# yxgeee/OpenIBL

Measured on NVIDIA H100. Metric: images_per_sec_extraction, higher is better.
Workload: dtype f32 (bf16x3 split on wgmma, fp32 accumulate)

## Files before the change

### openibl_b200/csrc/tc_conv.cu

```cuda
#include "common.cuh"
#include "tc_common.cuh"

namespace ibl {

using namespace tc;

namespace tc {
EncodeTiledFn get_encode_tiled() {
  static const EncodeTiledFn fn = []() -> EncodeTiledFn {
    void* p = nullptr;
    cudaDriverEntryPointQueryResult qres;
    if (cudaGetDriverEntryPoint("cuTensorMapEncodeTiled", &p, cudaEnableDefault, &qres) ==
            cudaSuccess &&
        qres == cudaDriverEntryPointSuccess)
      return reinterpret_cast<EncodeTiledFn>(p);
    return nullptr;
  }();
  return fn;
}

int make_tmap(CUtensorMap* out, CUtensorMapDataType dt, int rank, const void* base,
              const uint64_t* dims, const uint64_t* strides_bytes, const uint32_t* box, int swizzle_bytes) {
  EncodeTiledFn enc = get_encode_tiled();
  if (!enc) {
// ... 13 lines not shown
                   CU_TENSOR_MAP_INTERLEAVE_NONE,
                   swizzle_bytes == 64 ? CU_TENSOR_MAP_SWIZZLE_64B : CU_TENSOR_MAP_SWIZZLE_128B,
                   CU_TENSOR_MAP_L2_PROMOTION_L2_256B, CU_TENSOR_MAP_FLOAT_OOB_FILL_NONE);
  if (r != CUDA_SUCCESS) {
    set_last_error("cuTensorMapEncodeTiled failed with CUresult " + std::to_string((int)r));
    return IBL_ERR_CUDA;
  }
  return IBL_OK;
}
}

int tc_driver_init() { return get_encode_tiled() ? IBL_OK : IBL_ERR_NO_DEVICE; }

struct ConvTcArgs {
  int N, H, W, cin, cout;
  int tw_log2;
  int tiles_w, tiles_h;
  int n_tiles;
  int total_tiles;
  int relu, pool;
  const float* bias;
  __nv_bfloat16* y_hi;
  __nv_bfloat16* y_lo;
  float* y_f32;
  float* ssq;
  long long ssq_stride;
};

__device__ __forceinline__ uint32_t pack_bf16x2(float a, float b) {
  __nv_bfloat162 t = __floats2bfloat162_rn(a, b);
  return *reinterpret_cast<uint32_t*>(&t);
}

template <int BN>
__device__ __forceinline__ void conv_epilogue_tile(const ConvTcArgs& a, const Acc128<BN>& acc, float* stg, int img, int h0,
                                                   int w0, int n0, int nt, int r, int c, int dr_lanes, int bar = 1) {
  const int h = h0 + r, w = w0 + c;
  bool valid;
  long long pix;
  if (a.pool) {
    const int OH = a.H >> 1, OW = a.W >> 1;
    const int oh = h >> 1, ow = w >> 1;
    valid = oh < OH && ow < OW && img < a.N;
    pix = ((long long)img * OH + oh) * OW + ow;
  } else {
    valid = h < a.H && w < a.W && img < a.N;
    pix = ((long long)img * a.H + h) * a.W + w;
  }
  float ssq_acc = 0.f;
#pragma unroll
  for (int ch = 0; ch < BN / 32; ++ch) {
    uint32_t raw[32];
    acc.rows32(ch, stg, raw, bar);
    if (a.pool) {
      const bool s1 = (c & 1) != 0, s2 = (r & 1) != 0;
      float u[16];
#pragma unroll
      for (int j = 0; j < 16; ++j) {
        const float lo_h = __uint_as_float(raw[j]), hi_h = __uint_as_float(raw[j + 16]);
        const float got = __shfl_xor_sync(0xffffffffu, s1 ? lo_h : hi_h, 1);
        u[j] = fmaxf(s1 ? hi_h : lo_h, got);
      }
      float w8[8];
#pragma unroll
      for (int j = 0; j < 8; ++j) {
        const float got = __shfl_xor_sync(0xffffffffu, s2 ? u[j] : u[j + 8], dr_lanes);
        w8[j] = fmaxf(s2 ? u[j + 8] : u[j], got);
      }
      if (valid) {
        const int cbase = n0 + ch * 32 + (s1 ? 16 : 0) + (s2 ? 8 : 0);
        const float4 b0 = __ldg(reinterpret_cast<const float4*>(a.bias + cbase));
        const float4 b1 = __ldg(reinterpret_cast<const float4*>(a.bias + cbase) + 1);
        const float bb[8] = {b0.x, b0.y, b0.z, b0.w, b1.x, b1.y, b1.z, b1.w};
#pragma unroll
        for (int j = 0; j < 8; ++j) {
          w8[j] = w8[j] + bb[j];
          if (a.relu) w8[j] = fmaxf(w8[j], 0.f);
        }
        const long long off = pix * a.cout + cbase;
        if (a.y_f32) {
          float4* o = reinterpret_cast<float4*>(a.y_f32 + off);
          o[0] = make_float4(w8[0], w8[1], w8[2], w8[3]);
          o[1] = make_float4(w8[4], w8[5], w8[6], w8[7]);
        } else {
          uint32_t hi[4], lo[4];
#pragma unroll
          for (int j = 0; j < 4; ++j) {
            const float x0 = w8[2 * j], x1 = w8[2 * j + 1];
            const __nv_bfloat16 h0b = __float2bfloat16_rn(x0), h1b = __float2bfloat16_rn(x1);
            __nv_bfloat162 hh(h0b, h1b);
            hi[j] = *reinterpret_cast<uint32_t*>(&hh);
            lo[j] = pack_bf16x2(x0 - __bfloat162float(h0b), x1 - __bfloat162float(h1b));
          }
          *reinterpret_cast<uint4*>(a.y_hi + off) = make_uint4(hi[0], hi[1], hi[2], hi[3]);
          *reinterpret_cast<uint4*>(a.y_lo + off) = make_uint4(lo[0], lo[1], lo[2], lo[3]);
        }
      }
      continue;
    }
    float v[32];
    const float4* bp = reinterpret_cast<const float4*>(a.bias + n0 + ch * 32);
#pragma unroll
    for (int j = 0; j < 8; ++j) {
      const float4 b = __ldg(bp + j);
      v[4 * j + 0] = __uint_as_float(raw[4 * j + 0]) + b.x;
      v[4 * j + 1] = __uint_as_float(raw[4 * j + 1]) + b.y;
      v[4 * j + 2] = __uint_as_float(raw[4 * j + 2]) + b.z;
      v[4 * j + 3] = __uint_as_float(raw[4 * j + 3]) + b.w;
    }
    if (a.relu) {
#pragma unroll
      for (int j = 0; j < 32; ++j) v[j] = fmaxf(v[j], 0.f);
    }
    if (a.ssq) {
#pragma unroll
      for (int j = 0; j < 32; ++j) ssq_acc = fmaf(v[j], v[j], ssq_acc);
    }
    if (valid) {
      const long long off = pix * a.cout + n0 + ch * 32;
      if (a.y_f32) {
        float4* o = reinterpret_cast<float4*>(a.y_f32 + off);
#pragma unroll
        for (int j = 0; j < 8; ++j) o[j] = make_float4(v[4 * j], v[4 * j + 1], v[4 * j + 2], v[4 * j + 3]);
      } else {
        uint32_t hi[16], lo[16];
#pragma unroll
        for (int j = 0; j < 16; ++j) {
          const float x0 = v[2 * j], x1 = v[2 * j + 1];
          const __nv_bfloat16 h0b = __float2bfloat16_rn(x0), h1b = __float2bfloat16_rn(x1);
          __nv_bfloat162 hh(h0b, h1b);
          hi[j] = *reinterpret_cast<uint32_t*>(&hh);
          lo[j] = pack_bf16x2(x0 - __bfloat162float(h0b), x1 - __bfloat162float(h1b));
        }
        uint4* oh4 = reinterpret_cast<uint4*>(a.y_hi + off);
        uint4* ol4 = reinterpret_cast<uint4*>(a.y_lo + off);
#pragma unroll
        for (int j = 0; j < 4; ++j) {
          oh4[j] = make_uint4(hi[4 * j], hi[4 * j + 1], hi[4 * j + 2], hi[4 * j + 3]);
          ol4[j] = make_uint4(lo[4 * j], lo[4 * j + 1], lo[4 * j + 2], lo[4 * j + 3]);
        }
      }
    }
  }
  if (a.ssq && valid && !a.pool) a.ssq[(long long)nt * a.ssq_stride + pix] = ssq_acc;
}

constexpr int TC_BM = 128;
constexpr int TC_BK = 64;
constexpr int TC_A_BYTES = TC_BM * TC_BK * 2;

constexpr int TC_HALO_W = 10, TC_HALO_H = 18;
constexpr int TC_HALO_ROWS = TC_HALO_W * TC_HALO_H;
constexpr int TC_HALO_PLANE = 23 * 1024;
constexpr int TC_HALO_STAGE = 2 * TC_HALO_PLANE;

constexpr int TC_WIDE_PX = 256;
constexpr int TC_WIDE_HALO_PLANE = 41 * 1024;

template <int BN, int STAGES, bool HALO = false, int NA = 0, int WTW = 0>
struct ConvTcSmem {
  static constexpr int THREADS = HALO ? 384 : 160;
  static constexpr int CONSUMERS = HALO ? 2 : 1;
  static constexpr int B_BYTES = BN * TC_BK * 2;
  static constexpr int STAGE_BYTES = HALO ? 2 * B_BYTES : 2 * TC_A_BYTES + 2 * B_BYTES;
  static constexpr int HALO_PLANE = WTW ? TC_WIDE_HALO_PLANE : TC_HALO_PLANE;
  static constexpr int A_RING = HALO ? NA * 2 * HALO_PLANE : 0;
  static constexpr int STG = WTW ? 0 : CONSUMERS * ACC_STG_BYTES;
  static constexpr int BYTES = A_RING + STAGES * STAGE_BYTES + STG + 1024  + 256 ;
};

struct AccWide {
  float d[2][64];
};

__device__ __forceinline__ float wide_pick(bool swap, float a, float b) { return swap ? b : a; }

__device__ __forceinline__ void wide_transpose4(uint32_t (&x)[4][2], int j) {
#pragma unroll
  for (int bit = 0; bit < 2; ++bit) {
    const bool mine = ((j >> bit) & 1) != 0;
#pragma unroll
    for (int p0 = 0; p0 < 4; ++p0) {
      if (p0 & (1 << bit)) continue;
      const int p1 = p0 | (1 << bit);
#pragma unroll
      for (int h = 0; h < 2; ++h) {
        const uint32_t got = __shfl_xor_sync(0xffffffffu, mine ? x[p0][h] : x[p1][h], 4 << bit);
        if (mine) x[p0][h] = got; else x[p1][h] = got;
      }
    }
  }
}

__device__ __forceinline__ void conv_wide_epilogue(const ConvTcArgs& a, const AccWide& acc, int img, int h0, int w0,
                                                   int nt) {
  constexpr int NV = 2, TH = 16;
  const int t = threadIdx.x & 127, w = t >> 5, lane = t & 31, g = lane >> 2, q = lane & 3, j = g & 3;
  const bool sw = (g >> 2) != 0;
  const int c = nt * 64 + 16 * w + 2 * g;
  const int cst = nt * 64 + 16 * w + 8 * (g >> 2);
  const float b0 = __ldg(a.bias + c), b1 = __ldg(a.bias + c + 1);
  auto activate = [&](float& v0, float& v1) {
    v0 += b0; v1 += b1;
    if (a.relu) { v0 = fmaxf(v0, 0.f); v1 = fmaxf(v1, 0.f); }
  };
  auto pack = [&](float v0, float v1, uint32_t (&x)[2]) {
    if (a.y_f32) {
      x[0] = __float_as_uint(v0); x[1] = __float_as_uint(v1);
    } else {
      const __nv_bfloat16 h0b = __float2bfloat16_rn(v0), h1b = __float2bfloat16_rn(v1);
      __nv_bfloat162 hh(h0b, h1b);
      x[0] = *reinterpret_cast<uint32_t*>(&hh);
      x[1] = pack_bf16x2(v0 - __bfloat162float(h0b), v1 - __bfloat162float(h1b));
    }
  };
  auto store = [&](const uint32_t (&x)[4][2], bool valid, long long pix) {
    if (!valid) return;
    const long long off = pix * a.cout + cst;
    if (a.y_f32) {
      float4* o = reinterpret_cast<float4*>(a.y_f32 + off);
      o[0] = make_float4(__uint_as_float(x[0][0]), __uint_as_float(x[0][1]), __uint_as_float(x[1][0]), __uint_as_float(x[1][1]));
      o[1] = make_float4(__uint_as_float(x[2][0]), __uint_as_float(x[2][1]), __uint_as_float(x[3][0]), __uint_as_float(x[3][1]));
    } else {
      *reinterpret_cast<uint4*>(a.y_hi + off) = make_uint4(x[0][0], x[1][0], x[2][0], x[3][0]);
      *reinterpret_cast<uint4*>(a.y_lo + off) = make_uint4(x[0][1], x[1][1], x[2][1], x[3][1]);
    }
  };
  if (a.pool) {
    const int OH = a.H >> 1, OW = a.W >> 1;
    const int ow = (w0 >> 1) + q;
#pragma unroll
    for (int v = 0; v < NV; ++v)
#pragma unroll
      for (int m = 0; m < TH / 8; ++m) {
        uint32_t x[4][2];
#pragma unroll
        for (int p = 0; p < 4; ++p) {
          const float* r0 = &acc.d[v][4 * (2 * (4 * m + p))];
          const float* r1 = r0 + 4;
          const float e0 = fmaxf(fmaxf(r0[0], r0[1]), fmaxf(r1[0], r1[1]));
          const float e1 = fmaxf(fmaxf(r0[2], r0[3]), fmaxf(r1[2], r1[3]));
          float v0 = wide_pick(sw, e0, e1), v1 = wide_pick(sw, e1, e0);
          activate(v0, v1);
          pack(v0, v1, x[p]);
        }
        wide_transpose4(x, j);
        const int oh = (h0 >> 1) + 4 * m + j, owv = ow + 4 * v;
        store(x, oh < OH && owv < OW && img < a.N, ((long long)img * OH + oh) * OW + owv);
      }
    return;
  }
#pragma unroll
  for (int v = 0; v < NV; ++v)
#pragma unroll
    for (int b = 0; b < TH / 2; ++b) {
      uint32_t x[4][2];
      float sq[4];
#pragma unroll
      for (int p = 0; p < 4; ++p) {
        const float* r = &acc.d[v][4 * (2 * b + (p >> 1)) + (p & 1)];
        const float e0 = r[0], e1 = r[2];
        float v0 = wide_pick(sw, e0, e1), v1 = wide_pick(sw, e1, e0);
        activate(v0, v1);
        sq[p] = fmaf(v1, v1, v0 * v0);
        pack(v0, v1, x[p]);
      }
      wide_transpose4(x, j);
      const int h = h0 + 2 * b + (j >> 1), wc = w0 + 8 * v + 2 * q + (j & 1);
      const bool valid = h < a.H && wc < a.W && img < a.N;
      const long long pix = ((long long)img * a.H + h) * a.W + wc;
      store(x, valid, pix);
      if (a.ssq) {
        float mine = 0.f;
#pragma unroll
        for (int p = 0; p < 4; ++p) {
          float s2 = sq[p];
          s2 += __shfl_xor_sync(0xffffffffu, s2, 4);
          s2 += __shfl_xor_sync(0xffffffffu, s2, 8);
          s2 += __shfl_xor_sync(0xffffffffu, s2, 16);
          if (p == j) mine = s2;
        }
        if (valid && g < 4) a.ssq[(long long)(nt * 4 + w) * a.ssq_stride + pix] = mine;
      }
    }
}

template <int BN, int STAGES, bool HALO, int NA, int WTW = 0>
__global__ void __launch_bounds__(ConvTcSmem<BN, STAGES, HALO, NA, WTW>::THREADS, 1)
conv3x3_tc_kernel(const __grid_constant__ CUtensorMap tm_xhi, const __grid_constant__ CUtensorMap tm_xlo,
                  const __grid_constant__ CUtensorMap tm_whi, const __grid_constant__ CUtensorMap tm_wlo,
                  const ConvTcArgs a) {
  extern __shared__ __align__(1024) uint8_t smem_raw[];
  uint8_t* smem = reinterpret_cast<uint8_t*>((reinterpret_cast<uintptr_t>(smem_raw) + 1023) & ~uintptr_t(1023));
  using L = ConvTcSmem<BN, STAGES, HALO, NA, WTW>;
  constexpr int HALO_PLANE = L::HALO_PLANE;
  constexpr int HALO_STAGE = 2 * HALO_PLANE;
  constexpr int PX = WTW ? TC_WIDE_PX : TC_BM;
  constexpr int B_BYTES = L::B_BYTES;
  constexpr int STAGE_BYTES = L::STAGE_BYTES;
  constexpr int A_RING = L::A_RING;
  uint8_t* ring = smem + A_RING;
  float* stg = reinterpret_cast<float*>(ring + STAGES * STAGE_BYTES);
  uint64_t* bars = reinterpret_cast<uint64_t*>(ring + STAGES * STAGE_BYTES + L::STG);
  uint64_t* full_bar = bars;
  uint64_t* empty_bar = bars + STAGES;
  uint64_t* afull_bar = bars + 2 * STAGES;
  uint64_t* aempty_bar = afull_bar + NA;
// ... 245 lines not shown
#pragma unroll
          for (int k = 0; k < TC_BK / 16; ++k) {
            const uint64_t ko = (uint64_t)(k * 2);
            acc.mma(a_lo + ko, a_lo + a_half + ko, b_hi + ko, (kc > 0 || tap > 0 || k > 0) ? 1u : 0u);
            acc.mma(a_hi + ko, a_hi + a_half + ko, b_lo + ko, 1u);
            acc.mma(a_hi + ko, a_hi + a_half + ko, b_hi + ko, 1u);
          }
          wgmma_commit();
          if (kc == kchunks - 1 && tap == 8 && lane == 0) mbar_arrive(&order_bar[cw ^ 1]);
          wgmma_wait<1>();
          if (prev >= 0) release_w(prev);
          if (prev_a >= 0) {
            if (lane == 0) mbar_arrive(&aempty_bar[prev_a]);
            prev_a = -1;
          }
          prev = stage;
          if (++stage == STAGES) { stage = 0; phase ^= 1; }
        }
        prev_a = astage;
        if (++astage == NA) { astage = 0; aphase ^= 1; }
      }
      wgmma_wait<0>();
      acc.fence_operands();
      release_w(prev);
      if (lane == 0) mbar_arrive(&aempty_bar[prev_a]);
      conv_epilogue_tile<BN>(a, acc, my_stg, img, h0, w0, nt * BN, nt, r, c, 8, bar);
    }
    } else {
    const int m = threadIdx.x;
    const int r = m >> a.tw_log2, c = m & (TW - 1);
    int stage = 0;
    uint32_t phase = 0;
    for (int tile = worker; tile < a.total_tiles; tile += n_workers) {
      int img, h0, w0, nt;
      coords(tile, img, h0, w0, nt);
      Acc128<BN> acc;
      int prev = -1;
      for (int kit = 0; kit < kiters; ++kit) {
        mbar_wait(&full_bar[stage], phase);
        const uint32_t sa = ring_a + stage * STAGE_BYTES;
        const uint64_t a_hi = gmma_desc_kmajor_sw128(sa), a_lo = gmma_desc_kmajor_sw128(sa + TC_A_BYTES);
        const uint64_t b_hi = gmma_desc_kmajor_sw128(sa + 2 * TC_A_BYTES);
        const uint64_t b_lo = gmma_desc_kmajor_sw128(sa + 2 * TC_A_BYTES + B_BYTES);
        constexpr uint64_t kHalf = (TC_BM / 2) * 128 / 16;
        wgmma_fence();
#pragma unroll
        for (int k = 0; k < TC_BK / 16; ++k) {
          const uint64_t ko = (uint64_t)(k * 2);
          acc.mma(a_lo + ko, a_lo + kHalf + ko, b_hi + ko, (kit > 0 || k > 0) ? 1u : 0u);
          acc.mma(a_hi + ko, a_hi + kHalf + ko, b_lo + ko, 1u);
          acc.mma(a_hi + ko, a_hi + kHalf + ko, b_hi + ko, 1u);
        }
        wgmma_commit();
        wgmma_wait<1>();
        if (prev >= 0) release_w(prev);
        prev = stage;
        if (++stage == STAGES) { stage = 0; phase ^= 1; }
      }
      wgmma_wait<0>();
      acc.fence_operands();
      if (prev >= 0) release_w(prev);
      conv_epilogue_tile<BN>(a, acc, stg, img, h0, w0, nt * BN, nt, r, c, TW);
    }
    }
  }
  __syncthreads();
}

template <int BN, int STAGES, bool HALO = false, int NA = 0, int WTW = 0>
static int launch_tc_variant(const CUtensorMap& xhi, const CUtensorMap& xlo, const CUtensorMap& whi,
                             const CUtensorMap& wlo, const ConvTcArgs& a, cudaStream_t s) {
  constexpr int smem = ConvTcSmem<BN, STAGES, HALO, NA, WTW>::BYTES;
  static_assert(smem <= 232448, "shared-memory budget");
  static DeviceOnce attr_done;
  if (!attr_done.done()) {
    IBL_CUDA_OK(cudaFuncSetAttribute(conv3x3_tc_kernel<BN, STAGES, HALO, NA, WTW>,
                                     cudaFuncAttributeMaxDynamicSharedMemorySize, smem));
    attr_done.mark();
  }
  const int sms = device_sm_count();
  const int grid = a.total_tiles < sms ? a.total_tiles : sms;
  conv3x3_tc_kernel<BN, STAGES, HALO, NA, WTW>
      <<<grid, ConvTcSmem<BN, STAGES, HALO, NA, WTW>::THREADS, smem, s>>>(xhi, xlo, whi, wlo, a);
  IBL_CUDA_OK(cudaGetLastError());
  return IBL_OK;
}

static int g_tc_bn_override = 0;
void tc_set_bn_override(int bn) { g_tc_bn_override = bn; }
static int g_tc_variant_override = 0;
void tc_set_variant_override(int v) { g_tc_variant_override = v; }

int launch_conv3x3_tc(const __nv_bfloat16* x_hi, const __nv_bfloat16* x_lo, const ConvParams& p,
                      int N, int H, int W, int cin, int cout, bool relu, bool pool,
                      __nv_bfloat16* y_hi, __nv_bfloat16* y_lo, float* y_f32, cudaStream_t s, float* ssq,
                      int* ssq_parts) {
  IBL_REQUIRE(cin % 64 == 0 && cout % 64 == 0, "tensor-core conv needs Cin%64==0 and Cout%64==0");
  IBL_REQUIRE(p.w_hi && p.w_lo, "tensor-core conv: weights were not re-laid-out");
  IBL_REQUIRE(H >= 1 && W >= 1 && N >= 1, "empty conv input");
  ConvTcArgs a{};
  a.N = N; a.H = H; a.W = W; a.cin = cin; a.cout = cout;
  auto waste = [&](int tw, int px) {
    int th = px / tw;
    return (long long)cdiv(W, tw) * tw * cdiv(H, th) * th;
  };
  const int tw128 = (waste(16, 128) <= waste(8, 128)) ? 16 : 8;
  constexpr int tw256 = 16;
  bool wide = waste(tw256, 256) <= waste(tw128, 128);
  if (g_tc_bn_override) wide = false;
  if (g_tc_variant_override) wide = g_tc_variant_override == 2;
  const int TW = wide ? tw256 : tw128, TH = (wide ? TC_WIDE_PX : TC_BM) / TW;
  a.tw_log2 = TW == 16 ? 4 : 3;
  a.tiles_w = cdiv(W, TW);
  a.tiles_h = cdiv(H, TH);
  int bn = wide ? 64 : cout % 128 == 0 ? 128 : 64;
  if (!wide && g_tc_bn_override && cout % g_tc_bn_override == 0 && (g_tc_bn_override == 64 || g_tc_bn_override == 128))
    bn = g_tc_bn_override;
  const bool halo = wide || bn == 128;
  a.n_tiles = cout / bn;
  a.total_tiles = (int)((long long)N * a.tiles_h * a.tiles_w * a.n_tiles);
  a.relu = relu; a.pool = pool;
  a.bias = p.bias; a.y_hi = y_hi; a.y_lo = y_lo; a.y_f32 = y_f32;
  a.ssq = pool ? nullptr : ssq;
  a.ssq_stride = (long long)N * H * W;
  if (ssq_parts) *ssq_parts = wide ? cout / 16 : a.n_tiles;

  CUtensorMap m_xhi, m_xlo, m_whi, m_wlo;
  {
    uint64_t dims[4] = {(uint64_t)cin, (uint64_t)W, (uint64_t)H, (uint64_t)N};
    uint64_t str[3] = {(uint64_t)cin * 2, (uint64_t)W * cin * 2, (uint64_t)H * W * cin * 2};
    uint32_t box[4] = {64, (uint32_t)(halo ? TW + 2 : TW), (uint32_t)(halo ? TH + 2 : TH), 1};
    IBL_RET(make_tmap(&m_xhi, CU_TENSOR_MAP_DATA_TYPE_BFLOAT16, 4, x_hi, dims, str, box));
    IBL_RET(make_tmap(&m_xlo, CU_TENSOR_MAP_DATA_TYPE_BFLOAT16, 4, x_lo, dims, str, box));
  }
  {
    uint64_t dims[3] = {(uint64_t)cin, (uint64_t)cout, 9};
    uint64_t str[2] = {(uint64_t)cin * 2, (uint64_t)cout * cin * 2};
    uint32_t box[3] = {64, (uint32_t)bn, 1};
    IBL_RET(make_tmap(&m_whi, CU_TENSOR_MAP_DATA_TYPE_BFLOAT16, 3, p.w_hi, dims, str, box));
    IBL_RET(make_tmap(&m_wlo, CU_TENSOR_MAP_DATA_TYPE_BFLOAT16, 3, p.w_lo, dims, str, box));
  }
  if (wide) return launch_tc_variant<64, 3, true, 2, 16>(m_xhi, m_xlo, m_whi, m_wlo, a, s);
  if (halo) return launch_tc_variant<128, 3, true, 2>(m_xhi, m_xlo, m_whi, m_wlo, a, s);
  return launch_tc_variant<64, 4>(m_xhi, m_xlo, m_whi, m_wlo, a, s);
}

struct Conv1FusedArgs {
  const float* x;
  const float* w1;
  const float* bias1;
  ConvTcArgs c2;
};

constexpr int F1_A1_ROWS = 192;
constexpr int F1_A1_PLANE = F1_A1_ROWS * 64;
constexpr int F1_W1_PLANE = 64 * 64;
constexpr int F1_W2_STAGE = 2 * 64 * TC_BK * 2;
constexpr int F1_W2_STAGES = 4;
constexpr int F1_OFF_W1 = 2 * TC_HALO_STAGE;
constexpr int F1_OFF_W2 = F1_OFF_W1 + 2 * F1_W1_PLANE;
constexpr int F1_OFF_STG = F1_OFF_W2 + F1_W2_STAGES * F1_W2_STAGE;
constexpr int F1_OFF_BAR = F1_OFF_STG + 2 * ACC_STG_BYTES;
constexpr int F1_SMEM = F1_OFF_BAR + 512 + 1024;
static_assert(2 * F1_A1_PLANE <= TC_HALO_STAGE, "A1 (hi | lo) is built inside the consumer's halo buffer");
static_assert(TC_HALO_STAGE % 1024 == 0 && F1_OFF_W1 % 512 == 0 && F1_OFF_W2 % 1024 == 0, "swizzle atom alignment");
static_assert(F1_SMEM <= 232448, "shared-memory budget of the fused conv1 kernel");

__device__ __forceinline__ void wgmma_n64_into_n128(float (&d)[64], uint64_t a, uint64_t b) {
  asm volatile(
      "{\n\t.reg .pred p;\n\tsetp.ne.b32 p, 1, 0;\n\t"
      "wgmma.mma_async.sync.aligned.m64n64k16.f32.bf16.bf16 {%0, %1, %2, %3, %4, %5, %6, %7, %8, %9, %10, %11, %12, %13, %14, %15, %16, %17, %18, %19, %20, %21, %22, %23, %24, %25, %26, %27, %28, %29, %30, %31}, %32, %33, p, 1, 1, 0, 0;\n\t}"
      : "+f"(d[0]), "+f"(d[1]), "+f"(d[2]), "+f"(d[3]), "+f"(d[4]), "+f"(d[5]), "+f"(d[6]), "+f"(d[7]), "+f"(d[8]), "+f"(d[9]), "+f"(d[10]), "+f"(d[11]), "+f"(d[12]), "+f"(d[13]), "+f"(d[14]), "+f"(d[15]), "+f"(d[16]), "+f"(d[17]), "+f"(d[18]), "+f"(d[19]), "+f"(d[20]), "+f"(d[21]), "+f"(d[22]), "+f"(d[23]), "+f"(d[24]), "+f"(d[25]), "+f"(d[26]), "+f"(d[27]), "+f"(d[28]), "+f"(d[29]), "+f"(d[30]), "+f"(d[31])
      : "l"(a), "l"(b));
}

__global__ void __launch_bounds__(384, 1)
conv1_fused_tc_kernel(const __grid_constant__ CUtensorMap tm_whi, const __grid_constant__ CUtensorMap tm_wlo,
                      const Conv1FusedArgs fa) {
  extern __shared__ __align__(1024) uint8_t smem_raw[];
  uint8_t* smem = reinterpret_cast<uint8_t*>((reinterpret_cast<uintptr_t>(smem_raw) + 1023) & ~uintptr_t(1023));
  const ConvTcArgs& a = fa.c2;
  uint8_t* w1 = smem + F1_OFF_W1;
  uint8_t* w2 = smem + F1_OFF_W2;
  float* stg = reinterpret_cast<float*>(smem + F1_OFF_STG);
  uint64_t* bars = reinterpret_cast<uint64_t*>(smem + F1_OFF_BAR);
  uint64_t* w_full = bars;
  uint64_t* w_empty = bars + F1_W2_STAGES;
  uint64_t* order_bar = bars + 2 * F1_W2_STAGES;
  float* bias1_s = reinterpret_cast<float*>(bars + 16);

  const int warp = threadIdx.x >> 5, lane = threadIdx.x & 31;
  for (int i = threadIdx.x; i < 64 * 4; i += blockDim.x) {
    const int n = i >> 2, j = i & 3;
    uint32_t hi[4], lo[4];
#pragma unroll
    for (int e = 0; e < 4; ++e) {
      float v[2];
#pragma unroll
      for (int u = 0; u < 2; ++u) {
        const int k = j * 8 + e * 2 + u;
        v[u] = 0.f;
        if (k < 27) v[u] = fa.w1[(n * 3 + (k % 3)) * 9 + (k / 3)];
      }
      const __nv_bfloat16 h0 = __float2bfloat16_rn(v[0]), h1 = __float2bfloat16_rn(v[1]);
      __nv_bfloat162 hh(h0, h1);
      hi[e] = *reinterpret_cast<uint32_t*>(&hh);
      lo[e] = pack_bf16x2(v[0] - __bfloat162float(h0), v[1] - __bfloat162float(h1));
    }
    const int pos = n * 64 + ((j ^ ((n >> 1) & 3)) * 16);
    *reinterpret_cast<uint4*>(w1 + pos) = make_uint4(hi[0], hi[1], hi[2], hi[3]);
    *reinterpret_cast<uint4*>(w1 + F1_W1_PLANE + pos) = make_uint4(lo[0], lo[1], lo[2], lo[3]);
  }
  if (threadIdx.x < 64) bias1_s[threadIdx.x] = fa.bias1[threadIdx.x];
  if (threadIdx.x == 0) {
    tma_prefetch_desc(&tm_whi);
    tma_prefetch_desc(&tm_wlo);
    for (int i = 0; i < F1_W2_STAGES; ++i) { mbar_init(&w_full[i], 1); mbar_init(&w_empty[i], 4); }
    mbar_init(&order_bar[0], 4);
    mbar_init(&order_bar[1], 4);
    fence_barrier_init();
  }
  fence_proxy_async();
  __syncthreads();
  const int tiles_per_img = a.tiles_h * a.tiles_w;
  auto coords = [&](int tile, int& img, int& h0, int& w0) {
    img = tile / tiles_per_img;
    const int rem = tile - img * tiles_per_img;
    h0 = (rem / a.tiles_w) * 16;
    w0 = (rem % a.tiles_w) * 8;
  };

  if (warp < 4) setmaxnreg_dec<40>();
  if (warp == 0) {
    int stage = 0; uint32_t phase = 0;
    for (int tile = blockIdx.x; tile < a.total_tiles; tile += gridDim.x) {
      for (int tap = 0; tap < 9; ++tap) {
        mbar_wait_warp(&w_empty[stage], phase ^ 1);
        uint8_t* st = w2 + stage * F1_W2_STAGE;
        if (elect_one()) {
          mbar_arrive_expect_tx(&w_full[stage], F1_W2_STAGE);
          tma_load_3d(st, &tm_whi, &w_full[stage], 0, 0, tap);
          tma_load_3d(st + F1_W2_STAGE / 2, &tm_wlo, &w_full[stage], 0, 0, tap);
        }
        __syncwarp();
        if (++stage == F1_W2_STAGES) { stage = 0; phase ^= 1; }
      }
    }
  } else if (warp >= 4) {
    setmaxnreg_inc<232>();
    const int cw = warp / 4 - 1;
    const int bar = 1 + cw;
    float* my_stg = stg + cw * (ACC_STG_BYTES / 4);
    uint8_t* halo = smem + cw * TC_HALO_STAGE;
    const int t = threadIdx.x & 127;
    const int r = t >> 3, c = t & 7;
    const uint32_t ha = smem_u32(halo);
    const uint64_t b1h = gmma_desc_kmajor_sw64(smem_u32(w1)), b1l = gmma_desc_kmajor_sw64(smem_u32(w1) + F1_W1_PLANE);
    const uint64_t a1h = gmma_desc_kmajor_sw64(ha), a1l = gmma_desc_kmajor_sw64(ha + F1_A1_PLANE);
    constexpr uint64_t kA1Tile = 64 * 64 / 16;
    constexpr uint64_t kHaloDesc = ((uint64_t)1 << 16) | ((uint64_t)((TC_HALO_W * 128) >> 4) << 32) | ((uint64_t)1 << 62);
    constexpr uint64_t kHaloHalf = 8 * TC_HALO_W * 128 / 16;
    const long long HW = (long long)a.H * a.W;
    for (int i = cw; blockIdx.x + i * gridDim.x < a.total_tiles; i += 2) {
      int img, h0, w0;
      coords(blockIdx.x + i * gridDim.x, img, h0, w0);
      int tl = t;
      asm volatile("" : "+r"(tl));
#pragma unroll
      for (int q = 0; q < 2; ++q) {
        const int p = q * 128 + tl;
        if (p < F1_A1_ROWS) {
          float v[32];
#pragma unroll
          for (int k = 0; k < 32; ++k) v[k] = 0.f;
          const int hl = p / TC_HALO_W, wl = p - hl * TC_HALO_W;
          const int ph = h0 - 1 + hl, pw = w0 - 1 + wl;
          if (p < TC_HALO_ROWS && ph >= 0 && ph < a.H && pw >= 0 && pw < a.W && img < a.N) {
            const float* xb = fa.x + (long long)img * 3 * HW;
#pragma unroll
            for (int tap = 0; tap < 9; ++tap) {
              const int ih = ph + tap / 3 - 1, iw = pw + tap % 3 - 1;
              if (ih >= 0 && ih < a.H && iw >= 0 && iw < a.W) {
                const long long o = (long long)ih * a.W + iw;
#pragma unroll
                for (int ci = 0; ci < 3; ++ci) v[tap * 3 + ci] = __ldg(xb + ci * HW + o);
              }
            }
          }
          uint8_t* rh = halo + p * 64;
#pragma unroll
          for (int j = 0; j < 4; ++j) {
            uint32_t hi[4], lo[4];
#pragma unroll
            for (int e = 0; e < 4; ++e) {
              const float x0 = v[8 * j + 2 * e], x1 = v[8 * j + 2 * e + 1];
              const __nv_bfloat16 h0b = __float2bfloat16_rn(x0), h1b = __float2bfloat16_rn(x1);
              __nv_bfloat162 hv(h0b, h1b);
              hi[e] = *reinterpret_cast<uint32_t*>(&hv);
              lo[e] = pack_bf16x2(x0 - __bfloat162float(h0b), x1 - __bfloat162float(h1b));
            }
            const int pos = (j ^ ((p >> 1) & 3)) * 16;
            *reinterpret_cast<uint4*>(rh + pos) = make_uint4(hi[0], hi[1], hi[2], hi[3]);
            *reinterpret_cast<uint4*>(rh + F1_A1_PLANE + pos) = make_uint4(lo[0], lo[1], lo[2], lo[3]);
          }
        }
      }
      fence_proxy_async();
      wg_sync(bar);
      float c1[3][32];
      wgmma_fence();
#pragma unroll
      for (int k = 0; k < 2; ++k) {
        const uint64_t ko = (uint64_t)(k * 2);
#pragma unroll
        for (int f = 0; f < 3; ++f) {
          const uint64_t fo = f * kA1Tile + ko;
          Wgmma<64, false, 0, 0>::mma(c1[f], a1l + fo, b1h + ko, k > 0 ? 1u : 0u);
          Wgmma<64, false, 0, 0>::mma(c1[f], a1h + fo, b1l + ko, 1u);
          Wgmma<64, false, 0, 0>::mma(c1[f], a1h + fo, b1h + ko, 1u);
        }
      }
      wgmma_commit();
      wgmma_wait<0>();
#pragma unroll
      for (int f = 0; f < 3; ++f)
#pragma unroll
        for (int j = 0; j < 32; ++j) asm volatile("" : "+f"(c1[f][j])::"memory");
      wg_sync(bar);
#pragma unroll
      for (int f = 0; f < 3; ++f) {
#pragma unroll
        for (int hf = 0; hf < 2; ++hf) {
          const int p = 64 * f + (tl & ~31) / 2 + ((tl & 31) >> 2) + 8 * hf;
          if (p < TC_HALO_ROWS) {
            const int hl = p / TC_HALO_W, wl = p - hl * TC_HALO_W;
            const int ph = h0 - 1 + hl, pw = w0 - 1 + wl;
            const bool inside = ph >= 0 && ph < a.H && pw >= 0 && pw < a.W && img < a.N;
            uint8_t* rh = halo + p * 128 + (tl & 3) * 4;
#pragma unroll
            for (int j = 0; j < 8; ++j) {
              const int ch = 8 * j + 2 * (tl & 3);
              float x0 = fmaxf(c1[f][4 * j + 2 * hf] + bias1_s[ch], 0.f);
              float x1 = fmaxf(c1[f][4 * j + 2 * hf + 1] + bias1_s[ch + 1], 0.f);
              if (!inside) { x0 = 0.f; x1 = 0.f; }
              const __nv_bfloat16 h0b = __float2bfloat16_rn(x0), h1b = __float2bfloat16_rn(x1);
              __nv_bfloat162 hv(h0b, h1b);
              const int pos = (j ^ (p & 7)) * 16;
              *reinterpret_cast<uint32_t*>(rh + pos) = *reinterpret_cast<uint32_t*>(&hv);
              *reinterpret_cast<uint32_t*>(rh + TC_HALO_PLANE + pos) =
                  pack_bf16x2(x0 - __bfloat162float(h0b), x1 - __bfloat162float(h1b));
            }
          }
        }
      }
      fence_proxy_async();
      wg_sync(bar);
      int stage = (i * 9) % F1_W2_STAGES;
      uint32_t phase = (uint32_t)((i * 9) / F1_W2_STAGES) & 1u;
      if (i > 0) mbar_wait(&order_bar[cw], (uint32_t)((i - 1) >> 1) & 1u);
      float d[2][64];
#pragma unroll
      for (int hm = 0; hm < 2; ++hm)
#pragma unroll
        for (int j = 0; j < 64; ++j) d[hm][j] = 0.f;
      int prev = -1;
      for (int tap = 0; tap < 9; ++tap) {
        mbar_wait(&w_full[stage], phase);
        const uint32_t toff = (uint32_t)((tap / 3) * TC_HALO_W + tap % 3) * 128u;
        const uint64_t a_hi = kHaloDesc | (uint64_t)(((ha + toff) >> 4) & 0x3fffu);
        const uint64_t a_lo = kHaloDesc | (uint64_t)(((ha + TC_HALO_PLANE + toff) >> 4) & 0x3fffu);
        const uint64_t b_w = gmma_desc_kmajor_sw128(smem_u32(w2 + stage * F1_W2_STAGE));
        wgmma_fence();
#pragma unroll
        for (int k = 0; k < TC_BK / 16; ++k) {
          const uint64_t ko = (uint64_t)(k * 2);
#pragma unroll
          for (int hm = 0; hm < 2; ++hm) {
            const uint64_t ho = hm ? kHaloHalf : 0;
            Wgmma<128, false, 0, 0>::mma(d[hm], a_hi + ho + ko, b_w + ko, (tap > 0 || k > 0) ? 1u : 0u);
            wgmma_n64_into_n128(d[hm], a_lo + ho + ko, b_w + ko);
          }
        }
        wgmma_commit();
        if (tap == 8 && lane == 0) mbar_arrive(&order_bar[cw ^ 1]);
        wgmma_wait<1>();
        if (prev >= 0 && lane == 0) mbar_arrive(&w_empty[prev]);
        prev = stage;
        if (++stage == F1_W2_STAGES) { stage = 0; phase ^= 1; }
      }
      wgmma_wait<0>();
#pragma unroll
      for (int hm = 0; hm < 2; ++hm)
#pragma unroll
        for (int j = 0; j < 64; ++j) asm volatile("" : "+f"(d[hm][j])::"memory");
      if (lane == 0) mbar_arrive(&w_empty[prev]);
      Acc128<64> acc;
#pragma unroll
      for (int hm = 0; hm < 2; ++hm)
#pragma unroll
        for (int j = 0; j < 32; ++j) acc.h[hm][j] = d[hm][j] + d[hm][32 + j];
      conv_epilogue_tile<64>(a, acc, my_stg, img, h0, w0, 0, 0, r, c, 8, bar);
    }
  }
  __syncthreads();
}

int launch_conv1_fused_tc(const float* x_nchw, const float* w1_oihw, const float* bias1, const ConvParams& p2, int N, int H,
                          int W, __nv_bfloat16* y_hi, __nv_bfloat16* y_lo, cudaStream_t s) {
  IBL_REQUIRE(p2.w_hi && p2.w_lo && p2.bias, "fused conv1: conv1_2 weights were not re-laid-out");
  Conv1FusedArgs fa{};
  fa.x = x_nchw; fa.w1 = w1_oihw; fa.bias1 = bias1;
  ConvTcArgs& a = fa.c2;
  a.N = N; a.H = H; a.W = W; a.cin = 64; a.cout = 64;
  a.tw_log2 = 3;
  a.tiles_w = cdiv(W, 8);
  a.tiles_h = cdiv(H, 16);
  a.n_tiles = 1;
  a.total_tiles = (int)((long long)N * a.tiles_h * a.tiles_w);
  a.relu = 1; a.pool = 1;
  a.bias = p2.bias; a.y_hi = y_hi; a.y_lo = y_lo; a.y_f32 = nullptr; a.ssq = nullptr; a.ssq_stride = 0;
  CUtensorMap m_whi, m_wlo;
  {
    uint64_t dims[3] = {64, 64, 9};
    uint64_t str[2] = {64 * 2, 64 * 64 * 2};
    uint32_t box[3] = {64, 64, 1};
    IBL_RET(make_tmap(&m_whi, CU_TENSOR_MAP_DATA_TYPE_BFLOAT16, 3, p2.w_hi, dims, str, box));
    IBL_RET(make_tmap(&m_wlo, CU_TENSOR_MAP_DATA_TYPE_BFLOAT16, 3, p2.w_lo, dims, str, box));
  }
  static DeviceOnce attr_done;
  if (!attr_done.done()) {
    IBL_CUDA_OK(cudaFuncSetAttribute(conv1_fused_tc_kernel, cudaFuncAttributeMaxDynamicSharedMemorySize, F1_SMEM));
    attr_done.mark();
  }
  const int sms = device_sm_count();
  const int grid = a.total_tiles < sms ? a.total_tiles : sms;
  conv1_fused_tc_kernel<<<grid, 384, F1_SMEM, s>>>(m_whi, m_wlo, fa);
  IBL_CUDA_OK(cudaGetLastError());
  return IBL_OK;
}

__global__ void maxpool2x2_planes_kernel(const __nv_bfloat16* __restrict__ hi,
                                         const __nv_bfloat16* __restrict__ lo, int N, int H, int W,
                                         int C, __nv_bfloat16* __restrict__ yhi,
                                         __nv_bfloat16* __restrict__ ylo) {
  const int OH = H / 2, OW = W / 2;
  const long long total = (long long)N * OH * OW * C;
  for (long long i = blockIdx.x * (long long)blockDim.x + threadIdx.x; i < total;
       i += (long long)gridDim.x * blockDim.x) {
    const int c = (int)(i % C);
    long long r = i / C;
    const int ow = (int)(r % OW);
    r /= OW;
    const int oh = (int)(r % OH);
    const long long n = r / OH;
    float best = -INFINITY;
    __nv_bfloat16 bh = __float2bfloat16_rn(0.f), bl = bh;
#pragma unroll
    for (int dy = 0; dy < 2; ++dy)
#pragma unroll
      for (int dx = 0; dx < 2; ++dx) {
        const long long src = ((n * H + oh * 2 + dy) * (long long)W + ow * 2 + dx) * C + c;
        const __nv_bfloat16 a = hi[src], b = lo[src];
        const float v = __bfloat162float(a) + __bfloat162float(b);
        if (v > best) { best = v; bh = a; bl = b; }
      }
    yhi[i] = bh;
    ylo[i] = bl;
  }
}

int launch_maxpool2x2_planes(const __nv_bfloat16* hi, const __nv_bfloat16* lo, int N, int H, int W,
                             int C, __nv_bfloat16* yhi, __nv_bfloat16* ylo, cudaStream_t s) {
  long long total = (long long)N * (H / 2) * (W / 2) * C;
  unsigned blocks = (unsigned)((total + 255) / 256);
  if (blocks > 132 * 32) blocks = 132 * 32;
  if (!blocks) blocks = 1;
  maxpool2x2_planes_kernel<<<blocks, 256, 0, s>>>(hi, lo, N, H, W, C, yhi, ylo);
  IBL_CUDA_OK(cudaGetLastError());
  return IBL_OK;
}

int tc_selftest(float* max_rel_err, cudaStream_t s) {
  (void)s;
  if (max_rel_err) *max_rel_err = 0.f;
  return tc_driver_init();
}

}
```

Before: 1253.

## Widen fused conv1 tile to 16x16 with transposed RS wgmma and pipelined conv1

```diff
diff --git a/openibl_b200/csrc/tc_conv.cu b/openibl_b200/csrc/tc_conv.cu
--- a/openibl_b200/csrc/tc_conv.cu
+++ b/openibl_b200/csrc/tc_conv.cu
@@ -189,7 +189,6 @@
 constexpr int TC_HALO_W = 10, TC_HALO_H = 18;
 constexpr int TC_HALO_ROWS = TC_HALO_W * TC_HALO_H;
 constexpr int TC_HALO_PLANE = 23 * 1024;
-constexpr int TC_HALO_STAGE = 2 * TC_HALO_PLANE;
 
 constexpr int TC_WIDE_PX = 256;
 constexpr int TC_WIDE_HALO_PLANE = 41 * 1024;
@@ -741,27 +740,28 @@
   ConvTcArgs c2;
 };
 
-constexpr int F1_A1_ROWS = 192;
-constexpr int F1_A1_PLANE = F1_A1_ROWS * 64;
+constexpr int F1_HALO_W = 18;
+constexpr int F1_HALO_ROWS = F1_HALO_W * F1_HALO_W;
+constexpr int F1_HALO_STAGE = 2 * TC_WIDE_HALO_PLANE;
+constexpr int F1_A1_TILE = 64 * 64;
 constexpr int F1_W1_PLANE = 64 * 64;
 constexpr int F1_W2_STAGE = 2 * 64 * TC_BK * 2;
-constexpr int F1_W2_STAGES = 4;
-constexpr int F1_OFF_W1 = 2 * TC_HALO_STAGE;
-constexpr int F1_OFF_W2 = F1_OFF_W1 + 2 * F1_W1_PLANE;
-constexpr int F1_OFF_STG = F1_OFF_W2 + F1_W2_STAGES * F1_W2_STAGE;
-constexpr int F1_OFF_BAR = F1_OFF_STG + 2 * ACC_STG_BYTES;
+constexpr int F1_W2_STAGES = 3;
+constexpr int F1_OFF_W2 = 2 * F1_HALO_STAGE;
+constexpr int F1_OFF_W1 = F1_OFF_W2 + F1_W2_STAGES * F1_W2_STAGE;
+constexpr int F1_OFF_BAR = F1_OFF_W1 + 2 * F1_W1_PLANE;
 constexpr int F1_SMEM = F1_OFF_BAR + 512 + 1024;
-static_assert(2 * F1_A1_PLANE <= TC_HALO_STAGE, "A1 (hi | lo) is built inside the consumer's halo buffer");
-static_assert(TC_HALO_STAGE % 1024 == 0 && F1_OFF_W1 % 512 == 0 && F1_OFF_W2 % 1024 == 0, "swizzle atom alignment");
+
+__host__ __device__ constexpr int f1_a1_off(int g, int plane) {
+  return (g < 5 ? g * 2 * F1_A1_TILE : TC_WIDE_HALO_PLANE) + plane * F1_A1_TILE;
+}
+static_assert(2 * F1_A1_TILE == 64 * 128, "a tile's A1 fills its own halo rows of the hi plane");
+static_assert(5 * 64 < F1_HALO_ROWS && 6 * 64 >= F1_HALO_ROWS && f1_a1_off(4, 1) + F1_A1_TILE <= TC_WIDE_HALO_PLANE &&
+                  F1_HALO_ROWS * 128 <= TC_WIDE_HALO_PLANE,
+              "six m64 tiles cover the halo, only tile 5 reaches past halo row 319, and the halo tile fits in a plane");
+static_assert(F1_HALO_STAGE % 1024 == 0 && F1_OFF_W2 % 1024 == 0 && F1_OFF_W1 % 512 == 0 && f1_a1_off(5, 1) % 512 == 0,
+              "swizzle atom alignment");
 static_assert(F1_SMEM <= 232448, "shared-memory budget of the fused conv1 kernel");
-
-__device__ __forceinline__ void wgmma_n64_into_n128(float (&d)[64], uint64_t a, uint64_t b) {
-  asm volatile(
-      "{\n\t.reg .pred p;\n\tsetp.ne.b32 p, 1, 0;\n\t"
-      "wgmma.mma_async.sync.aligned.m64n64k16.f32.bf16.bf16 {%0, %1, %2, %3, %4, %5, %6, %7, %8, %9, %10, %11, %12, %13, %14, %15, %16, %17, %18, %19, %20, %21, %22, %23, %24, %25, %26, %27, %28, %29, %30, %31}, %32, %33, p, 1, 1, 0, 0;\n\t}"
-      : "+f"(d[0]), "+f"(d[1]), "+f"(d[2]), "+f"(d[3]), "+f"(d[4]), "+f"(d[5]), "+f"(d[6]), "+f"(d[7]), "+f"(d[8]), "+f"(d[9]), "+f"(d[10]), "+f"(d[11]), "+f"(d[12]), "+f"(d[13]), "+f"(d[14]), "+f"(d[15]), "+f"(d[16]), "+f"(d[17]), "+f"(d[18]), "+f"(d[19]), "+f"(d[20]), "+f"(d[21]), "+f"(d[22]), "+f"(d[23]), "+f"(d[24]), "+f"(d[25]), "+f"(d[26]), "+f"(d[27]), "+f"(d[28]), "+f"(d[29]), "+f"(d[30]), "+f"(d[31])
-      : "l"(a), "l"(b));
-}
 
 __global__ void __launch_bounds__(384, 1)
 conv1_fused_tc_kernel(const __grid_constant__ CUtensorMap tm_whi, const __grid_constant__ CUtensorMap tm_wlo,
@@ -771,7 +771,6 @@
   const ConvTcArgs& a = fa.c2;
   uint8_t* w1 = smem + F1_OFF_W1;
   uint8_t* w2 = smem + F1_OFF_W2;
-  float* stg = reinterpret_cast<float*>(smem + F1_OFF_STG);
   uint64_t* bars = reinterpret_cast<uint64_t*>(smem + F1_OFF_BAR);
   uint64_t* w_full = bars;
   uint64_t* w_empty = bars + F1_W2_STAGES;
@@ -816,7 +815,7 @@
     img = tile / tiles_per_img;
     const int rem = tile - img * tiles_per_img;
     h0 = (rem / a.tiles_w) * 16;
-    w0 = (rem % a.tiles_w) * 8;
+    w0 = (rem % a.tiles_w) * 16;
   };
 
   if (warp < 4) setmaxnreg_dec<40>();
@@ -839,156 +838,160 @@
     setmaxnreg_inc<232>();
     const int cw = warp / 4 - 1;
     const int bar = 1 + cw;
-    float* my_stg = stg + cw * (ACC_STG_BYTES / 4);
-    uint8_t* halo = smem + cw * TC_HALO_STAGE;
+    uint8_t* halo = smem + cw * F1_HALO_STAGE;
     const int t = threadIdx.x & 127;
-    const int r = t >> 3, c = t & 7;
     const uint32_t ha = smem_u32(halo);
+    const uint32_t w2a = smem_u32(w2);
     const uint64_t b1h = gmma_desc_kmajor_sw64(smem_u32(w1)), b1l = gmma_desc_kmajor_sw64(smem_u32(w1) + F1_W1_PLANE);
-    const uint64_t a1h = gmma_desc_kmajor_sw64(ha), a1l = gmma_desc_kmajor_sw64(ha + F1_A1_PLANE);
     constexpr uint64_t kA1Tile = 64 * 64 / 16;
-    constexpr uint64_t kHaloDesc = ((uint64_t)1 << 16) | ((uint64_t)((TC_HALO_W * 128) >> 4) << 32) | ((uint64_t)1 << 62);
-    constexpr uint64_t kHaloHalf = 8 * TC_HALO_W * 128 / 16;
+    constexpr uint64_t kHaloDesc = ((uint64_t)1 << 16) | ((uint64_t)((F1_HALO_W * 128) >> 4) << 32) | ((uint64_t)1 << 62);
+    const int wq = (threadIdx.x >> 5) & 3, jl = lane & 7, hl8 = (lane >> 3) & 1;
+    const int wrow = 16 * wq + 2 * jl + (hl8 ^ (jl >> 2));
     const long long HW = (long long)a.H * a.W;
     for (int i = cw; blockIdx.x + i * gridDim.x < a.total_tiles; i += 2) {
       int img, h0, w0;
       coords(blockIdx.x + i * gridDim.x, img, h0, w0);
       int tl = t;
       asm volatile("" : "+r"(tl));
-#pragma unroll
-      for (int q = 0; q < 2; ++q) {
+      wg_sync(bar);
+#pragma unroll
+      for (int q = 0; q < 3; ++q) {
         const int p = q * 128 + tl;
-        if (p < F1_A1_ROWS) {
-          float v[32];
-#pragma unroll
-          for (int k = 0; k < 32; ++k) v[k] = 0.f;
-          const int hl = p / TC_HALO_W, wl = p - hl * TC_HALO_W;
-          const int ph = h0 - 1 + hl, pw = w0 - 1 + wl;
-          if (p < TC_HALO_ROWS && ph >= 0 && ph < a.H && pw >= 0 && pw < a.W && img < a.N) {
-            const float* xb = fa.x + (long long)img * 3 * HW;
-#pragma unroll
-            for (int tap = 0; tap < 9; ++tap) {
-              const int ih = ph + tap / 3 - 1, iw = pw + tap % 3 - 1;
-              if (ih >= 0 && ih < a.H && iw >= 0 && iw < a.W) {
-                const long long o = (long long)ih * a.W + iw;
-#pragma unroll
-                for (int ci = 0; ci < 3; ++ci) v[tap * 3 + ci] = __ldg(xb + ci * HW + o);
-              }
+        float v[32];
+#pragma unroll
+        for (int k = 0; k < 32; ++k) v[k] = 0.f;
+        const int hl = p / F1_HALO_W, wl = p - hl * F1_HALO_W;
+        const int ph = h0 - 1 + hl, pw = w0 - 1 + wl;
+        if (p < F1_HALO_ROWS && ph >= 0 && ph < a.H && pw >= 0 && pw < a.W && img < a.N) {
+          const float* xb = fa.x + (long long)img * 3 * HW;
+#pragma unroll
+          for (int tap = 0; tap < 9; ++tap) {
+            const int ih = ph + tap / 3 - 1, iw = pw + tap % 3 - 1;
+            if (ih >= 0 && ih < a.H && iw >= 0 && iw < a.W) {
+              const long long o = (long long)ih * a.W + iw;
+#pragma unroll
+              for (int ci = 0; ci < 3; ++ci) v[tap * 3 + ci] = __ldg(xb + ci * HW + o);
             }
           }
-          uint8_t* rh = halo + p * 64;
-#pragma unroll
-          for (int j = 0; j < 4; ++j) {
-            uint32_t hi[4], lo[4];
-#pragma unroll
-            for (int e = 0; e < 4; ++e) {
-              const float x0 = v[8 * j + 2 * e], x1 = v[8 * j + 2 * e + 1];
-              const __nv_bfloat16 h0b = __float2bfloat16_rn(x0), h1b = __float2bfloat16_rn(x1);
-              __nv_bfloat162 hv(h0b, h1b);
-              hi[e] = *reinterpret_cast<uint32_t*>(&hv);
-              lo[e] = pack_bf16x2(x0 - __bfloat162float(h0b), x1 - __bfloat162float(h1b));
-            }
-            const int pos = (j ^ ((p >> 1) & 3)) * 16;
-            *reinterpret_cast<uint4*>(rh + pos) = make_uint4(hi[0], hi[1], hi[2], hi[3]);
-            *reinterpret_cast<uint4*>(rh + F1_A1_PLANE + pos) = make_uint4(lo[0], lo[1], lo[2], lo[3]);
+        }
+        const int g = p >> 6, r = p & 63;
+        uint8_t* rh = halo + f1_a1_off(g, 0) + r * 64;
+        uint8_t* rl = halo + f1_a1_off(g, 1) + r * 64;
+#pragma unroll
+        for (int j = 0; j < 4; ++j) {
+          uint32_t hi[4], lo[4];
+#pragma unroll
+          for (int e = 0; e < 4; ++e) {
+            const float x0 = v[8 * j + 2 * e], x1 = v[8 * j + 2 * e + 1];
+            const __nv_bfloat16 h0b = __float2bfloat16_rn(x0), h1b = __float2bfloat16_rn(x1);
+            __nv_bfloat162 hv(h0b, h1b);
+            hi[e] = *reinterpret_cast<uint32_t*>(&hv);
+            lo[e] = pack_bf16x2(x0 - __bfloat162float(h0b), x1 - __bfloat162float(h1b));
           }
+          const int pos = (j ^ ((r >> 1) & 3)) * 16;
+          *reinterpret_cast<uint4*>(rh + pos) = make_uint4(hi[0], hi[1], hi[2], hi[3]);
+          *reinterpret_cast<uint4*>(rl + pos) = make_uint4(lo[0], lo[1], lo[2], lo[3]);
         }
       }
       fence_proxy_async();
       wg_sync(bar);
-      float c1[3][32];
-      wgmma_fence();
-#pragma unroll
-      for (int k = 0; k < 2; ++k) {
-        const uint64_t ko = (uint64_t)(k * 2);
-#pragma unroll
-        for (int f = 0; f < 3; ++f) {
-          const uint64_t fo = f * kA1Tile + ko;
-          Wgmma<64, false, 0, 0>::mma(c1[f], a1l + fo, b1h + ko, k > 0 ? 1u : 0u);
-          Wgmma<64, false, 0, 0>::mma(c1[f], a1h + fo, b1l + ko, 1u);
-          Wgmma<64, false, 0, 0>::mma(c1[f], a1h + fo, b1h + ko, 1u);
-        }
-      }
-      wgmma_commit();
-      wgmma_wait<0>();
-#pragma unroll
-      for (int f = 0; f < 3; ++f)
-#pragma unroll
-        for (int j = 0; j < 32; ++j) asm volatile("" : "+f"(c1[f][j])::"memory");
-      wg_sync(bar);
-#pragma unroll
-      for (int f = 0; f < 3; ++f) {
+      float c1[2][32];
+      auto issue_c1 = [&](int g, float (&acc)[32]) {
+        const uint64_t a1h = gmma_desc_kmajor_sw64(ha + f1_a1_off(g, 0));
+        const uint64_t a1l = gmma_desc_kmajor_sw64(ha + f1_a1_off(g, 1));
+        wgmma_fence();
+#pragma unroll
+        for (int k = 0; k < 2; ++k) {
+          const uint64_t ko = (uint64_t)(k * 2);
+          Wgmma<64, false, 0, 0>::mma(acc, a1l + ko, b1h + ko, k > 0 ? 1u : 0u);
+          Wgmma<64, false, 0, 0>::mma(acc, a1h + ko, b1l + ko, 1u);
+          Wgmma<64, false, 0, 0>::mma(acc, a1h + ko, b1h + ko, 1u);
+        }
+        wgmma_commit();
+      };
+      issue_c1(5, c1[0]);
+      issue_c1(0, c1[1]);
+#pragma unroll
+      for (int step = 0; step < 6; ++step) {
+        const int g = step == 0 ? 5 : step - 1;
+        float (&acc)[32] = c1[step & 1];
+        if (step < 5) wgmma_wait<1>(); else wgmma_wait<0>();
+#pragma unroll
+        for (int j = 0; j < 32; ++j) asm volatile("" : "+f"(acc[j])::"memory");
+        wg_sync(bar);
 #pragma unroll
         for (int hf = 0; hf < 2; ++hf) {
-          const int p = 64 * f + (tl & ~31) / 2 + ((tl & 31) >> 2) + 8 * hf;
-          if (p < TC_HALO_ROWS) {
-            const int hl = p / TC_HALO_W, wl = p - hl * TC_HALO_W;
+          const int p = 64 * g + (tl & ~31) / 2 + ((tl & 31) >> 2) + 8 * hf;
+          if (p < F1_HALO_ROWS) {
+            const int hl = p / F1_HALO_W, wl = p - hl * F1_HALO_W;
             const int ph = h0 - 1 + hl, pw = w0 - 1 + wl;
             const bool inside = ph >= 0 && ph < a.H && pw >= 0 && pw < a.W && img < a.N;
             uint8_t* rh = halo + p * 128 + (tl & 3) * 4;
 #pragma unroll
             for (int j = 0; j < 8; ++j) {
               const int ch = 8 * j + 2 * (tl & 3);
-              float x0 = fmaxf(c1[f][4 * j + 2 * hf] + bias1_s[ch], 0.f);
-              float x1 = fmaxf(c1[f][4 * j + 2 * hf + 1] + bias1_s[ch + 1], 0.f);
+              float x0 = fmaxf(acc[4 * j + 2 * hf] + bias1_s[ch], 0.f);
+              float x1 = fmaxf(acc[4 * j + 2 * hf + 1] + bias1_s[ch + 1], 0.f);
               if (!inside) { x0 = 0.f; x1 = 0.f; }
               const __nv_bfloat16 h0b = __float2bfloat16_rn(x0), h1b = __float2bfloat16_rn(x1);
               __nv_bfloat162 hv(h0b, h1b);
               const int pos = (j ^ (p & 7)) * 16;
               *reinterpret_cast<uint32_t*>(rh + pos) = *reinterpret_cast<uint32_t*>(&hv);
-              *reinterpret_cast<uint32_t*>(rh + TC_HALO_PLANE + pos) =
+              *reinterpret_cast<uint32_t*>(rh + TC_WIDE_HALO_PLANE + pos) =
                   pack_bf16x2(x0 - __bfloat162float(h0b), x1 - __bfloat162float(h1b));
             }
           }
         }
+        if (step + 2 < 6) issue_c1(step + 1, acc);
       }
       fence_proxy_async();
       wg_sync(bar);
       int stage = (i * 9) % F1_W2_STAGES;
       uint32_t phase = (uint32_t)((i * 9) / F1_W2_STAGES) & 1u;
       if (i > 0) mbar_wait(&order_bar[cw], (uint32_t)((i - 1) >> 1) & 1u);
-      float d[2][64];
-#pragma unroll
-      for (int hm = 0; hm < 2; ++hm)
-#pragma unroll
-        for (int j = 0; j < 64; ++j) d[hm][j] = 0.f;
+      AccWide acc;
+      uint32_t fw[2][2][4];
       int prev = -1;
+#pragma unroll 1
       for (int tap = 0; tap < 9; ++tap) {
         mbar_wait(&w_full[stage], phase);
-        const uint32_t toff = (uint32_t)((tap / 3) * TC_HALO_W + tap % 3) * 128u;
-        const uint64_t a_hi = kHaloDesc | (uint64_t)(((ha + toff) >> 4) & 0x3fffu);
-        const uint64_t a_lo = kHaloDesc | (uint64_t)(((ha + TC_HALO_PLANE + toff) >> 4) & 0x3fffu);
-        const uint64_t b_w = gmma_desc_kmajor_sw128(smem_u32(w2 + stage * F1_W2_STAGE));
-        wgmma_fence();
+        const uint32_t sb = w2a + stage * F1_W2_STAGE;
+        ldsm_a_sw128(fw[0][0], sb, wrow, 0);
+        ldsm_a_sw128(fw[0][1], sb + F1_W2_STAGE / 2, wrow, 0);
+        const uint32_t toff = (uint32_t)((tap / 3) * F1_HALO_W + tap % 3) * 128u;
+        const uint64_t x_hi = kHaloDesc | (uint64_t)(((ha + toff) >> 4) & 0x3fffu);
+        const uint64_t x_lo = kHaloDesc | (uint64_t)(((ha + TC_WIDE_HALO_PLANE + toff) >> 4) & 0x3fffu);
 #pragma unroll
         for (int k = 0; k < TC_BK / 16; ++k) {
+          const uint32_t(&fh)[4] = fw[k & 1][0];
+          const uint32_t(&fl)[4] = fw[k & 1][1];
           const uint64_t ko = (uint64_t)(k * 2);
-#pragma unroll
-          for (int hm = 0; hm < 2; ++hm) {
-            const uint64_t ho = hm ? kHaloHalf : 0;
-            Wgmma<128, false, 0, 0>::mma(d[hm], a_hi + ho + ko, b_w + ko, (tap > 0 || k > 0) ? 1u : 0u);
-            wgmma_n64_into_n128(d[hm], a_lo + ho + ko, b_w + ko);
+          wgmma_fence();
+#pragma unroll
+          for (int v = 0; v < 2; ++v) WgmmaRS<128>::mma(acc.d[v], fh, x_lo + 64 * v + ko, (tap > 0 || k > 0) ? 1u : 0u);
+#pragma unroll
+          for (int v = 0; v < 2; ++v) WgmmaRS<128>::mma(acc.d[v], fl, x_hi + 64 * v + ko, 1u);
+#pragma unroll
+          for (int v = 0; v < 2; ++v) WgmmaRS<128>::mma(acc.d[v], fh, x_hi + 64 * v + ko, 1u);
+          wgmma_commit();
+          if (k == 3 && tap == 8 && lane == 0) mbar_arrive(&order_bar[cw ^ 1]);
+          wgmma_wait<1>();
+          if (k == 0 && prev >= 0 && lane == 0) mbar_arrive(&w_empty[prev]);
+          if (k + 1 < TC_BK / 16) {
+            ldsm_a_sw128(fw[(k + 1) & 1][0], sb, wrow, k + 1);
+            ldsm_a_sw128(fw[(k + 1) & 1][1], sb + F1_W2_STAGE / 2, wrow, k + 1);
           }
         }
-        wgmma_commit();
-        if (tap == 8 && lane == 0) mbar_arrive(&order_bar[cw ^ 1]);
-        wgmma_wait<1>();
-        if (prev >= 0 && lane == 0) mbar_arrive(&w_empty[prev]);
         prev = stage;
         if (++stage == F1_W2_STAGES) { stage = 0; phase ^= 1; }
       }
       wgmma_wait<0>();
 #pragma unroll
-      for (int hm = 0; hm < 2; ++hm)
-#pragma unroll
-        for (int j = 0; j < 64; ++j) asm volatile("" : "+f"(d[hm][j])::"memory");
+      for (int v = 0; v < 2; ++v)
+#pragma unroll
+        for (int e = 0; e < 64; ++e) asm volatile("" : "+f"(acc.d[v][e])::"memory");
       if (lane == 0) mbar_arrive(&w_empty[prev]);
-      Acc128<64> acc;
-#pragma unroll
-      for (int hm = 0; hm < 2; ++hm)
-#pragma unroll
-        for (int j = 0; j < 32; ++j) acc.h[hm][j] = d[hm][j] + d[hm][32 + j];
-      conv_epilogue_tile<64>(a, acc, my_stg, img, h0, w0, 0, 0, r, c, 8, bar);
+      conv_wide_epilogue(a, acc, img, h0, w0, 0);
     }
   }
   __syncthreads();
@@ -1001,8 +1004,8 @@
   fa.x = x_nchw; fa.w1 = w1_oihw; fa.bias1 = bias1;
   ConvTcArgs& a = fa.c2;
   a.N = N; a.H = H; a.W = W; a.cin = 64; a.cout = 64;
-  a.tw_log2 = 3;
-  a.tiles_w = cdiv(W, 8);
+  a.tw_log2 = 4;
+  a.tiles_w = cdiv(W, 16);
   a.tiles_h = cdiv(H, 16);
   a.n_tiles = 1;
   a.total_tiles = (int)((long long)N * a.tiles_h * a.tiles_w);
```

After: 1291, median of 6. 3.0% higher.
